# wangheda/youtube-8m

Hardware: AMD Instinct MI355X
Metric: training videos/sec (higher is better)
Workload: dtype f32; 1 GPU; BASELINE configs[3]: LstmModel (2 x BasicLSTMCell(1024), dynamic_rnn over F=300) on raw uint8 [B,300,1152] frames + MoeModel head (2 mixtures, V=4716), fp32 training step (fwd+bwd+clip+Adam); per_gpu_batch=128, global_batch=128, frames=300, parallelism=dp1, params=113902808

## Files before the change

### include/yt8m_hip.h

```cpp
#ifndef YT8M_HIP_H
#define YT8M_HIP_H
#include <stdint.h>

#ifdef __cplusplus
extern "C" {
#endif

typedef void* yt8m_stream_t;

enum yt8m_status { YT8M_OK = 0, YT8M_E_BADARG = -1, YT8M_E_SHAPE = -2, YT8M_E_HIP = -3, YT8M_E_RCCL = -4 };
enum yt8m_label_dtype { YT8M_LABEL_U8 = 0, YT8M_LABEL_F32 = 1 };

int yt8m_abi_version(void);
const char* yt8m_last_error(void);
const char* yt8m_built_arch(void);

int yt8m_prof_enable(int on);
int yt8m_prof_reset(void);
int yt8m_prof_get(int family, int64_t* launches, double* total_ms);
int yt8m_prof_get_flops(int family, double* flops);
int yt8m_prof_get_bytes(int family, double* bytes);

int yt8m_probe_mfma_f32(int iters, int blocks, float* sink, yt8m_stream_t stream);
int yt8m_probe_mfma_bf16(int iters, int blocks, int random_operands, float* sink, yt8m_stream_t stream);
int yt8m_probe_copy_f32(const float* src, float* dst, int64_t n, yt8m_stream_t stream);
int yt8m_probe_placement(int* out, int blocks, int spin_ticks, yt8m_stream_t stream);
int yt8m_stream_create_cu_mask(const uint32_t* mask, int words, yt8m_stream_t* stream);
int yt8m_stream_destroy(yt8m_stream_t stream);

int yt8m_gemm_f32(int transA, int transB, int64_t M, int64_t N, int64_t K,
                  const float* A, int64_t lda, const float* B, int64_t ldb,
                  float* C, int64_t ldc, const float* bias, float beta, yt8m_stream_t stream);

int yt8m_gemm_f32_batched(int transA, int transB, int64_t M, int64_t N, int64_t K,
                          const float* A, int64_t lda, int64_t strideA, const float* B, int64_t ldb, int64_t strideB,
                          float* C, int64_t ldc, int64_t strideC, float beta, int64_t batch, yt8m_stream_t stream);

typedef struct yt8m_gemm_problem {
  int64_t M, N, K;
  const void* A; int64_t lda;
  const void* B; int64_t ldb;
  float* C; int64_t ldc;
  const float* bias;
  float beta;
} yt8m_gemm_problem;
int64_t yt8m_gemm_workspace_bytes(void);
int yt8m_gemm_f32_grouped(int transA, int transB, int nprob, const yt8m_gemm_problem* probs, void* workspace,
                          int64_t workspace_bytes, yt8m_stream_t stream);
int yt8m_gemm_bf16_nt_grouped(int nprob, const yt8m_gemm_problem* probs, void* workspace, int64_t workspace_bytes,
                              yt8m_stream_t stream);
int64_t yt8m_x3_image_bytes(int64_t rows, int64_t K);
int yt8m_x3_split(const float* src, int64_t R, int64_t C, int64_t ld, float scale, void* plain, void* trans, yt8m_stream_t stream);
int yt8m_gemm_x3_nt_grouped(int nprob, const yt8m_gemm_problem* probs, void* workspace, int64_t workspace_bytes,
                            yt8m_stream_t stream);
int yt8m_h2_split(const float* src, int64_t R, int64_t C, int64_t ld, float scale, const float* dscale, void* plain, void* trans,
                  float* colpart, yt8m_stream_t stream);
int yt8m_h2_absmax(const float* src, int64_t R, int64_t C, int64_t ld, void* word, yt8m_stream_t stream);
int yt8m_h2_degraded(uint64_t* counts, int reset, yt8m_stream_t stream);
int yt8m_h2_split_dropout(const float* src, int64_t R, int64_t C, float scale, const float* dscale, void* plain, void* trans,
                          float keep_prob, uint64_t seed, int64_t offset, yt8m_stream_t stream);
int yt8m_h2_split_rowmax(const float* src, int64_t R, int64_t C, int64_t ld, const void* rowmax, float* inv, void* plain,
                         yt8m_stream_t stream);
int yt8m_h2_split_ex(const float* src, int64_t R, int64_t C, int64_t ld, float scale, const void* dscale, const float* rowscale, void* plain,
                     void* trans, void* trans_scaled, float* colpart, float* colpart_scaled, yt8m_stream_t stream);
int yt8m_gemm_h1x2_nt_ex(int64_t M, int64_t N, int64_t K, const void* A1, int64_t ska, const void* B2, int64_t skb, float* C, int64_t ldc,
                         const float* bias, float alpha, const void* dsb, const float* rowscale, const float* colsum, float colsum_scale,
                         float beta, void* workspace, int64_t workspace_bytes, yt8m_stream_t stream);
int yt8m_h2_rowscales(const float* src, int64_t R, int64_t C, int64_t ld, float* S, float* inv, yt8m_stream_t stream);
int yt8m_h2_split_rows(const float* src, int64_t R, int64_t C, int64_t ld, const float* S, void* plain, yt8m_stream_t stream);
int yt8m_gemm_h2_nt_ex(int64_t M, int64_t N, int64_t K, const void* A2, int64_t ska, const void* B2, int64_t skb, float* C, int64_t ldc,
                       const float* bias, float alpha, const void* dsa, const void* dsb, const float* rowscale, float beta, void* workspace,
                       int64_t workspace_bytes, yt8m_stream_t stream);
int yt8m_timepool_max_f32(const float* y, int64_t F, int64_t B, int64_t N, int64_t ldy, float* out, int32_t* idx, int64_t ldo,
                          yt8m_stream_t stream);
int yt8m_timepool_shiftmax_f32(const float* z, int64_t F, int64_t B, int64_t ldz, int nfilt, const int32_t* fs, const int32_t* ncol, float* out,
                               int32_t* idx, int64_t ldo, yt8m_stream_t stream);
int yt8m_u8_cnn_pool_dw(const uint8_t* q, const float* r_tm, const int32_t* idx, const float* g, int64_t ldg, int64_t B, int64_t F, int64_t D,
                        int64_t N, int64_t fs, float* dW, float beta, yt8m_stream_t stream);
int yt8m_f32_cnn_pool_dw(const float* x, int64_t ldx, const int32_t* idx, const float* g, int64_t ldg, int64_t B, int64_t F, int64_t D,
                         int64_t N, int64_t fs, float* dW, int64_t lddw, float beta, yt8m_stream_t stream);
int yt8m_f32_cnn_pool_dx(const int32_t* idx, const float* g, int64_t ldg, int64_t B, int64_t F, int64_t D, int nfilt, const float* const* wt,
                         const int32_t* fs, const int32_t* ncol, float* dx, int64_t lddx, yt8m_stream_t stream);
int yt8m_u8_frames_image_f16(const uint8_t* q, const int32_t* num_frames, int64_t B, int64_t F, int64_t D, float eps, void* image,
                             float* x_tm, float* r_out, yt8m_stream_t stream);
int yt8m_u8_frames_image_t_f16(const uint8_t* q, const int32_t* num_frames, int64_t B, int64_t F, int64_t D, void* image_t,
                               yt8m_stream_t stream);
int yt8m_gemm_h2_nt_grouped(int nprob, const yt8m_gemm_problem* probs, const float* alphas, const float* const* dsa,
                            const float* const* dsb, void* workspace, int64_t workspace_bytes, yt8m_stream_t stream);
int yt8m_x3_set_combine(int mode);
int yt8m_x3_set_schedule(int mode);
#define YT8M_GEMM_ROLE_DW 0x100
#define YT8M_GEMM_ROLE_H2 0x200
int yt8m_gemm_x3_pays(int64_t M, int64_t N, int64_t K);
int64_t yt8m_gemm_auto_scratch_bytes(int transA, int transB, int nprob, const yt8m_gemm_problem* probs);
int yt8m_gemm_auto_grouped(int transA, int transB, int nprob, const yt8m_gemm_problem* probs, void* workspace,
                           int64_t workspace_bytes, void* image_scratch, int64_t image_scratch_bytes, uint64_t* used_x3,
                           yt8m_stream_t stream);
int yt8m_gemm_auto_grouped_ex(int transA, int transB, int nprob, const yt8m_gemm_problem* probs, const float* const* absmaxA,
                              const float* const* absmaxB, void* workspace, int64_t workspace_bytes, void* image_scratch,
                              int64_t image_scratch_bytes, uint64_t* used_x3, yt8m_stream_t stream);
int yt8m_gemm_x1x3_nt(int64_t M, int64_t N, int64_t K, const void* A1, const void* B3, float* C, int64_t ldc, const float* bias,
                      const float* rowscale, const float* colsum, float colsum_scale, void* workspace, int64_t workspace_bytes,
                      yt8m_stream_t stream);
int yt8m_gemm_x1x3_nt_ex(int64_t M, int64_t N, int64_t K, const void* A1, int64_t ska, const void* B3, int64_t skb, float* C,
                         int64_t ldc, const float* bias, float alpha, const float* rowscale, const float* colsum,
                         float colsum_scale, float beta, void* workspace, int64_t workspace_bytes, yt8m_stream_t stream);
int yt8m_bf16_image(const float* src, int64_t R, int64_t C, int64_t ld, float scale, void* plain, void* trans, yt8m_stream_t stream);
int yt8m_gemm_b1_nt_grouped(int nprob, const yt8m_gemm_problem* probs, void* workspace, int64_t workspace_bytes, yt8m_stream_t stream);
int yt8m_gemm_b1_nt_grouped_bf16c(int nprob, const yt8m_gemm_problem* probs, unsigned c_bf16_mask, void* workspace, int64_t workspace_bytes,
                                  yt8m_stream_t stream);
int yt8m_moe_mix_fwd_bf16z(const void* Zg, const void* Ze, float* p, int64_t B, int64_t V, int M, yt8m_stream_t stream);
int yt8m_moe_mix_bwd_bf16_images_z16(const void* Zg, const void* Ze, const float* dp, const void* labels, int label_dtype, int64_t B,
                                     int64_t V, int M, float eps, float dscale, const float* upstream_dev, void* dZg_img, int64_t g_kb,
                                     void* dZg_t_img, int64_t gt_kb, void* dZe_img, int64_t e_kb, void* dZe_t_img, int64_t et_kb,
                                     float* be_part, yt8m_stream_t stream);
int yt8m_bf16_image_colsum(const float* src, int64_t R, int64_t C, int64_t ld, float scale, const float* rowscale, void* plain,
                           void* trans, void* trans_scaled, float* colpart, float* colpart_scaled, yt8m_stream_t stream);
int yt8m_gemm_b1_nt_ex(int64_t M, int64_t N, int64_t K, const void* A1, int64_t ska, const void* B1, int64_t skb, float* C, int64_t ldc,
                       const float* bias, float alpha, const float* rowscale, const float* colsum, float colsum_scale, float beta,
                       void* workspace, int64_t workspace_bytes, yt8m_stream_t stream);
int yt8m_x3_split_ex(const float* src, int64_t R, int64_t C, int64_t ld, float scale, const float* rowscale, void* plain,
                     void* trans, void* trans_scaled, yt8m_stream_t stream);
int yt8m_x3_split_colsum(const float* src, int64_t R, int64_t C, int64_t ld, float scale, const float* rowscale, void* plain,
                         void* trans, void* trans_scaled, float* colpart, float* colpart_scaled, yt8m_stream_t stream);
int yt8m_cast_f32_bf16(const float* src, int64_t rows, int64_t cols, int64_t ld, void* dst, int64_t dst_ld, int transpose,
                       yt8m_stream_t stream);
int yt8m_cast_f32_bf16_dual(const float* src, int64_t rows, int64_t cols, int64_t ld, void* dst_plain, int64_t plain_ld,
                            void* dst_trans, int64_t trans_ld, yt8m_stream_t stream);

int yt8m_l2norm_fwd_f32(const float* x, float* y, int64_t rows, int64_t cols, float eps, yt8m_stream_t stream);
int yt8m_l2norm_bwd_f32(const float* x, const float* dy, float* dx, int64_t rows, int64_t cols, float eps,
                        yt8m_stream_t stream);
int yt8m_dequant_l2norm_u8(const uint8_t* q, const int32_t* num_frames, float* x,
                           int64_t B, int64_t F, int64_t D, float eps, yt8m_stream_t stream);
int yt8m_dequant_mean_l2norm_u8(const uint8_t* q, const int32_t* num_frames, float* x,
                                int64_t B, int64_t F, int64_t D, float eps, yt8m_stream_t stream);
int yt8m_resolution_mean_u8(const uint8_t* q, const int32_t* num_frames, float* y, int32_t* num_frames_out, int64_t B, int64_t F,
                            int64_t D, int64_t resolution, int l2norm, float eps, yt8m_stream_t stream);
int yt8m_resolution_mean_f32(const float* x, const int32_t* num_frames, float* y, int32_t* num_frames_out, int64_t B, int64_t F,
                             int64_t D, int64_t resolution, int l2norm, float eps, yt8m_stream_t stream);
int yt8m_frame_pyramid_u8(const uint8_t* q, const int32_t* num_frames, int64_t B, int64_t F, int64_t D, int levels, int nseg,
                          const int64_t* widths, float* const* y, int32_t* const* num_frames_out, float eps, yt8m_stream_t stream);
int yt8m_frame_pyramid_supported(int64_t D, int nseg, const int64_t* widths, int levels);

int yt8m_moe_mix_fwd(const float* Zg, const float* Ze, float* p, int64_t B, int64_t V, int M,
                     yt8m_stream_t stream);
int yt8m_moe_mix_bwd(float* Zg, float* Ze, const float* dp, int64_t B, int64_t V, int M,
                     yt8m_stream_t stream);

int64_t yt8m_moe_mix_xent_workspace_bytes(int64_t B, int64_t V);
int yt8m_moe_mix_xent_fwd(const float* Zg, const float* Ze, const void* labels, int label_dtype, float* p,
                          float* loss_out, int64_t B, int64_t V, int M, float eps, void* workspace,
                          yt8m_stream_t stream);
int yt8m_moe_mix_xent_bwd(float* Zg, float* Ze, const void* labels, int label_dtype, const float* upstream_dev,
                          int64_t B, int64_t V, int M, float eps, float upstream, yt8m_stream_t stream);
int yt8m_moe_mix_xent_bwd_absmax(float* Zg, float* Ze, const void* labels, int label_dtype, const float* upstream_dev, int64_t B, int64_t V,
                                 int M, float eps, float upstream, void* absmax2, yt8m_stream_t stream);

int64_t yt8m_moe_workspace_bytes(int64_t B, int64_t V);
int64_t yt8m_moe_workspace_bytes_ex(int64_t B, int64_t D, int64_t V, int M);
int yt8m_moe_fwd(const float* x, const float* Wg, const float* We, const float* be, const void* labels, int label_dtype,
                 int64_t B, int64_t D, int64_t V, int M, float eps, float* Zg, float* Ze, float* p, float* loss_out,
                 void* workspace, int64_t workspace_bytes, yt8m_stream_t stream);
int yt8m_moe_bwd(const float* x, const float* Wg, const float* We, float* Zg, float* Ze, const void* labels, int label_dtype,
                 int64_t B, int64_t D, int64_t V, int M, float eps, float upstream, float* dWg, float* dWe, float* dbe,
                 float beta, float* dx, void* workspace, int64_t workspace_bytes, yt8m_stream_t stream);
int yt8m_logistic_fwd_bwd(const float* x, const float* W, const float* b, const void* labels, int label_dtype, int64_t B,
                          int64_t D, int64_t V, float eps, float* p, float* loss_out, float* Z, float* dW, float* db,
                          float beta, float* dx, void* workspace, int64_t workspace_bytes, yt8m_stream_t stream);

int yt8m_skinny_supported(int64_t M, int64_t K, int64_t N);
int64_t yt8m_skinny_workspace_bytes(int64_t M, int64_t K, int64_t N);
int yt8m_skinny_fwd_f32(const float* x, int64_t ldx, const float* W, int64_t ldw, const float* bias, float* y, int64_t ldy,
                        int64_t M, int64_t K, int64_t N, float beta, yt8m_stream_t stream);
int yt8m_skinny_dw_f32(const float* x, int64_t ldx, const float* dy, int64_t ldy, float* dW, int64_t lddw, int64_t M, int64_t K,
                       int64_t N, float beta, void* workspace, int64_t workspace_bytes, yt8m_stream_t stream);
int yt8m_skinny_dx_f32(const float* dy, int64_t ldy, const float* W, int64_t ldw, float* dx, int64_t lddx, int64_t M, int64_t K,
                       int64_t N, float beta, yt8m_stream_t stream);

int64_t yt8m_lstm_packed16_elems(int64_t B, int64_t H);
int yt8m_lstm_pack_bf16(const float* Wh, int64_t ldw, int64_t H, void* Wp16, void* Wq16, yt8m_stream_t stream);
int yt8m_lstm_steps_fwd_bf16(float* z, const void* Wp16, float* cs, float* hs, void* hs16, float* out, const int32_t* num_frames,
                             int64_t t0, int64_t T, int64_t B, int64_t H, float forget_bias, yt8m_stream_t stream);
// ... 409 lines not shown
```

### youtube-8m_amd/_lib.py

```python
import ctypes
import os

_HERE = os.path.dirname(os.path.abspath(__file__))
LIB_PATH = os.environ.get("YT8M_LIB", os.path.join(_HERE, "libyt8m_hip.so"))

c_void_p, c_int, c_int64, c_float, c_double = ctypes.c_void_p, ctypes.c_int, ctypes.c_int64, ctypes.c_float, ctypes.c_double
P = c_void_p

class GemmProblem(ctypes.Structure):
    _fields_ = [("M", c_int64), ("N", c_int64), ("K", c_int64), ("A", c_void_p), ("lda", c_int64), ("B", c_void_p),
                ("ldb", c_int64), ("C", c_void_p), ("ldc", c_int64), ("bias", c_void_p), ("beta", c_float)]


STREAM_HOOK = ctypes.CFUNCTYPE(None, ctypes.c_void_p, ctypes.c_void_p)


class PersistBwdImages(ctypes.Structure):
    _fields_ = [("plain", ctypes.c_void_p), ("trans", ctypes.c_void_p), ("trans_scaled", ctypes.c_void_p), ("rowscale", ctypes.c_void_p),
                ("colpart", ctypes.c_void_p), ("colpart_scaled", ctypes.c_void_p)]


class LstmStackDesc(ctypes.Structure):
    _fields_ = [("B", c_int64), ("F", c_int64), ("D", c_int64), ("H", c_int64), ("L", ctypes.c_int32), ("input_u8", ctypes.c_int32),
                ("forget_bias", c_float), ("fwd_chunks", ctypes.c_int32), ("bwd_chunks", ctypes.c_int32), ("need_dx", ctypes.c_int32),
                ("input_keep_prob", c_float), ("reserved0", ctypes.c_int32), ("dropout_seed", ctypes.c_uint64 * 8)]


class WimgDemand(ctypes.Structure):
    _fields_ = [("src", c_void_p), ("R", c_int64), ("C", c_int64), ("ld", c_int64), ("trans", ctypes.c_int32), ("planes", ctypes.c_int32),
                ("scale", c_float), ("pad", ctypes.c_int32)]


class WimgSpec(ctypes.Structure):
    _fields_ = [("plain", c_void_p), ("trans", c_void_p), ("row0", c_int64), ("rows", c_int64), ("scale", c_float),
                ("planes", ctypes.c_int32)]


class WimgJob(ctypes.Structure):
    _fields_ = [("offset", c_int64), ("R", c_int64), ("C", c_int64), ("tensor", ctypes.c_int32), ("nspec", ctypes.c_int32),
                ("tile_base", c_int64), ("spec", WimgSpec * 4)]


class OptRanges(ctypes.Structure):
    _fields_ = [("w", c_void_p), ("m", c_void_p), ("v", c_void_p), ("g", c_void_p), ("chunks", c_void_p), ("tensor_chunk_start", c_void_p),
                ("tensor_chunk_start_host", c_void_p), ("l2", c_void_p), ("partial", c_void_p), ("norms", c_void_p), ("skip_tensor", c_void_p),
                ("jobs", c_void_p), ("job_tensor_host", c_void_p), ("job_tile_base_host", c_void_p), ("njobs", ctypes.c_int32),
                ("nranges", ctypes.c_int32), ("range_lo", ctypes.c_int32 * 8), ("range_hi", ctypes.c_int32 * 8), ("gscale", c_float),
                ("clip", c_float), ("lr_t", c_float), ("beta1", c_float), ("beta2", c_float), ("eps", c_float), ("after_stream", c_void_p)]


DESC = ctypes.POINTER(LstmStackDesc)
PP = ctypes.POINTER(c_void_p)

SIGNATURES = {
    "yt8m_abi_version": (c_int, []),
    "yt8m_last_error": (ctypes.c_char_p, []),
    "yt8m_built_arch": (ctypes.c_char_p, []),
    "yt8m_prof_enable": (c_int, [c_int]),
    "yt8m_prof_reset": (c_int, []),
    "yt8m_prof_get": (c_int, [c_int, ctypes.POINTER(c_int64), ctypes.POINTER(c_double)]),
    "yt8m_prof_get_flops": (c_int, [c_int, ctypes.POINTER(c_double)]),
    "yt8m_prof_get_bytes": (c_int, [c_int, ctypes.POINTER(ctypes.c_double)]),
    "yt8m_probe_mfma_f32": (c_int, [c_int, c_int, P, P]),
    "yt8m_probe_mfma_bf16": (c_int, [c_int, c_int, c_int, P, P]),
    "yt8m_probe_copy_f32": (c_int, [P, P, c_int64, P]),
    "yt8m_probe_placement": (c_int, [P, c_int, c_int, P]),
    "yt8m_stream_create_cu_mask": (c_int, [P, c_int, ctypes.POINTER(P)]),
    "yt8m_stream_destroy": (c_int, [P]),
    "yt8m_gemm_f32": (c_int, [c_int, c_int, c_int64, c_int64, c_int64, P, c_int64, P, c_int64, P, c_int64, P, c_float, P]),
    "yt8m_gemm_workspace_bytes": (c_int64, []),
    "yt8m_gemm_f32_grouped": (c_int, [c_int, c_int, c_int, ctypes.POINTER(GemmProblem), P, c_int64, P]),
    "yt8m_gemm_bf16_nt_grouped": (c_int, [c_int, ctypes.POINTER(GemmProblem), P, c_int64, P]),
    "yt8m_gemm_x3_pays": (c_int, [c_int64, c_int64, c_int64]),
    "yt8m_gemm_auto_scratch_bytes": (c_int64, [c_int, c_int, c_int, ctypes.POINTER(GemmProblem)]),
    "yt8m_gemm_auto_grouped": (c_int, [c_int, c_int, c_int, ctypes.POINTER(GemmProblem), P, c_int64, P, c_int64, ctypes.POINTER(ctypes.c_uint64), P]),
    "yt8m_gemm_auto_grouped_ex": (c_int, [c_int, c_int, c_int, ctypes.POINTER(GemmProblem), ctypes.POINTER(ctypes.c_void_p), ctypes.POINTER(ctypes.c_void_p),
                                          P, c_int64, P, c_int64, ctypes.POINTER(ctypes.c_uint64), P]),
    "yt8m_x3_image_bytes": (c_int64, [c_int64, c_int64]),
    "yt8m_x3_split": (c_int, [P, c_int64, c_int64, c_int64, c_float, P, P, P]),
    "yt8m_gemm_x3_nt_grouped": (c_int, [c_int, ctypes.POINTER(GemmProblem), P, c_int64, P]),
    "yt8m_gemm_x1x3_nt": (c_int, [c_int64, c_int64, c_int64, P, P, P, c_int64, P, P, P, c_float, P, c_int64, P]),
    "yt8m_gemm_x1x3_nt_ex": (c_int, [c_int64, c_int64, c_int64, P, c_int64, P, c_int64, P, c_int64, P, c_float, P, P, c_float, c_float, P,
                                     c_int64, P]),
    "yt8m_bf16_image": (c_int, [P, c_int64, c_int64, c_int64, c_float, P, P, P]),
    "yt8m_gemm_b1_nt_grouped": (c_int, [c_int, ctypes.POINTER(GemmProblem), P, c_int64, P]),
    "yt8m_gemm_b1_nt_grouped_bf16c": (c_int, [c_int, ctypes.POINTER(GemmProblem), ctypes.c_uint, P, c_int64, P]),
    "yt8m_x3_split_ex": (c_int, [P, c_int64, c_int64, c_int64, c_float, P, P, P, P, P]),
    "yt8m_x3_split_colsum": (c_int, [P, c_int64, c_int64, c_int64, c_float, P, P, P, P, P, P, P]),
    "yt8m_x3_set_combine": (c_int, [c_int]),
    "yt8m_x3_set_schedule": (c_int, [c_int]),
    "yt8m_bf16_image_colsum": (c_int, [P, c_int64, c_int64, c_int64, c_float, P, P, P, P, P, P, P]),
    "yt8m_gemm_b1_nt_ex": (c_int, [c_int64, c_int64, c_int64, P, c_int64, P, c_int64, P, c_int64, P, c_float, P, P, c_float, c_float, P,
                                   c_int64, P]),
    "yt8m_u8_frames_image_t": (c_int, [P, P, c_int64, c_int64, c_int64, P, P]),
    "yt8m_lstm_stack_supported": (c_int, [DESC]),
    "yt8m_lstm_stack_tape_bytes": (c_int64, [DESC]),
    "yt8m_lstm_stack_scratch_bytes": (c_int64, [DESC]),
    "yt8m_lstm_stack_partition": (c_int, [DESC, ctypes.POINTER(c_int), ctypes.POINTER(c_int)]),
    "yt8m_lstm_stack_set_prep_hook": (c_int, [P, P]),
    "yt8m_lstm_stack_streams": (c_int, [c_int, PP, ctypes.POINTER(c_void_p)]),
    "yt8m_lstm_stack_fwd": (c_int, [DESC, P, P, PP, PP, P, c_int64, P, c_int64, P]),
    "yt8m_lstm_stack_view": (c_int, [DESC, P, c_int, c_int, ctypes.POINTER(c_void_p)]),
    "yt8m_lstm_stack_bwd": (c_int, [DESC, P, P, PP, P, c_int64, P, c_int64, P, PP, PP, PP, PP, ctypes.POINTER(c_float),
                                    ctypes.POINTER(c_float), P, P]),
    "yt8m_lstm_stack_status": (c_int, [DESC, P, P]),
    "yt8m_lstm_stack_layer_done_wait": (c_int, [c_int, P]),
    "yt8m_u8_frames_image": (c_int, [P, P, c_int64, c_int64, c_int64, c_float, P, P, P, P]),
    "yt8m_cast_f32_bf16": (c_int, [P, c_int64, c_int64, c_int64, P, c_int64, c_int, P]),
    "yt8m_cast_f32_bf16_dual": (c_int, [P, c_int64, c_int64, c_int64, P, c_int64, P, c_int64, P]),
    "yt8m_gemm_f32_batched": (c_int, [c_int, c_int, c_int64, c_int64, c_int64, P, c_int64, c_int64, P, c_int64, c_int64,
                                      P, c_int64, c_int64, c_float, c_int64, P]),
    "yt8m_l2norm_fwd_f32": (c_int, [P, P, c_int64, c_int64, c_float, P]),
    "yt8m_l2norm_bwd_f32": (c_int, [P, P, P, c_int64, c_int64, c_float, P]),
    "yt8m_dequant_l2norm_u8": (c_int, [P, P, P, c_int64, c_int64, c_int64, c_float, P]),
    "yt8m_dequant_mean_l2norm_u8": (c_int, [P, P, P, c_int64, c_int64, c_int64, c_float, P]),
    "yt8m_moe_workspace_bytes": (c_int64, [c_int64, c_int64]),
    "yt8m_moe_workspace_bytes_ex": (c_int64, [c_int64, c_int64, c_int64, c_int]),
    "yt8m_moe_fwd": (c_int, [P, P, P, P, P, c_int, c_int64, c_int64, c_int64, c_int, c_float, P, P, P, P, P, c_int64, P]),
    "yt8m_moe_bwd": (c_int, [P, P, P, P, P, P, c_int, c_int64, c_int64, c_int64, c_int, c_float, c_float, P, P, P, c_float, P, P,
                             c_int64, P]),
    "yt8m_logistic_fwd_bwd": (c_int, [P, P, P, P, c_int, c_int64, c_int64, c_int64, c_float, P, P, P, P, P, c_float, P, P,
                                      c_int64, P]),
    "yt8m_moe_mix_fwd": (c_int, [P, P, P, c_int64, c_int64, c_int, P]),
    "yt8m_moe_mix_bwd": (c_int, [P, P, P, c_int64, c_int64, c_int, P]),
    "yt8m_moe_mix_xent_workspace_bytes": (c_int64, [c_int64, c_int64]),
    "yt8m_moe_mix_xent_fwd": (c_int, [P, P, P, c_int, P, P, c_int64, c_int64, c_int, c_float, P, P]),
    "yt8m_moe_mix_xent_bwd": (c_int, [P, P, P, c_int, P, c_int64, c_int64, c_int, c_float, c_float, P]),
    "yt8m_moe_mix_xent_bwd_absmax": (c_int, [P, P, P, c_int, P, c_int64, c_int64, c_int, c_float, c_float, P, P]),
    "yt8m_skinny_supported": (c_int, [c_int64, c_int64, c_int64]),
    "yt8m_skinny_workspace_bytes": (c_int64, [c_int64, c_int64, c_int64]),
    "yt8m_skinny_fwd_f32": (c_int, [P, c_int64, P, c_int64, P, P, c_int64, c_int64, c_int64, c_int64, c_float, P]),
    "yt8m_skinny_dw_f32": (c_int, [P, c_int64, P, c_int64, P, c_int64, c_int64, c_int64, c_int64, c_float, P, c_int64, P]),
    "yt8m_skinny_dx_f32": (c_int, [P, c_int64, P, c_int64, P, c_int64, c_int64, c_int64, c_int64, c_float, P]),
    "yt8m_lstm_packed16_elems": (c_int64, [c_int64, c_int64]),
    "yt8m_lstm_pack_bf16": (c_int, [P, c_int64, c_int64, P, P, P]),
    "yt8m_lstm_steps_fwd_bf16": (c_int, [P, P, P, P, P, P, P, c_int64, c_int64, c_int64, c_int64, c_float, P]),
    "yt8m_lstm_steps_bwd_bf16": (c_int, [P, P, P, P, P, P, P, c_int, P, c_int64, c_int64, c_int64, c_int64, P]),
    "yt8m_u8_frame_scales": (c_int, [P, P, c_int64, c_int64, c_int64, c_float, P, P]),
    "yt8m_skinny_fwd_u8": (c_int, [P, c_int64, P, c_int64, P, P, P, P, c_int64, c_int64, c_int64, c_int64, c_float, P]),
    "yt8m_skinny_dw_u8": (c_int, [P, c_int64, P, c_int64, P, P, c_int64, c_int64, c_int64, c_int64, c_float, P, c_int64, P]),
    "yt8m_attn_pool_fwd_u8": (c_int, [P, P, P, P, c_int64, c_int64, c_int64, c_int64, P]),
    "yt8m_attn_pool_dw_u8": (c_int, [P, P, P, P, P, c_int64, c_int64, c_int64, c_int64, P]),
    "yt8m_attn_pool_supported": (c_int, [c_int64, c_int64, c_int64, c_int64]),
    "yt8m_attn_pool_fwd": (c_int, [P, P, P, c_int64, c_int64, c_int64, c_int64, P]),
    "yt8m_attn_pool_bwd": (c_int, [P, P, P, P, P, c_int64, c_int64, c_int64, c_int64, P]),
    "yt8m_gru_layer_fwd": (c_int, [P, P, P, c_int64, P, c_int64, P, P, P, P, c_int64, c_int64, c_int64, P, c_int64, P]),
    "yt8m_gru_layer_bwd": (c_int, [P, P, P, c_int64, P, c_int64, P, P, P, P, P, P, P, c_int64, c_int64, c_int64, P, c_int64, P]),
    "yt8m_lnlstm_layer_fwd": (c_int, [P, P, c_int64, P, P, P, P, P, P, P, c_int64, c_int64, c_int64, c_float, c_float,
                                      ctypes.c_uint64, P, c_int64, P]),
    "yt8m_lnlstm_layer_bwd": (c_int, [P, P, c_int64, P, P, P, P, P, P, P, P, P, P, P, P, c_int64, c_int64, c_int64, c_float,
                                      c_float, ctypes.c_uint64, P, c_int64, P]),
    "yt8m_dropout_f32": (c_int, [P, P, c_int64, c_float, ctypes.c_uint64, c_int64, P]),
    "yt8m_add_noise_f32": (c_int, [P, P, c_int64, c_float, ctypes.c_uint64, c_int64, P]),
    "yt8m_moe_mix_bwd_bf16_partial_rows": (c_int64, [c_int64]),
    "yt8m_moe_mix_bwd_bf16": (c_int, [P, P, P, P, c_int, c_int64, c_int64, c_int, c_float, c_float, P, P, c_int64, P, c_int64,
                                      P, c_int64, P, c_int64, P, P]),
    "yt8m_moe_mix_bwd_bf16_images": (c_int, [P, P, P, P, c_int, c_int64, c_int64, c_int, c_float, c_float, P, P, c_int64, P, c_int64,
                                      P, c_int64, P, c_int64, P, P]),
    "yt8m_moe_mix_bwd_bf16_images_z16": (c_int, [P, P, P, P, c_int, c_int64, c_int64, c_int, c_float, c_float, P, P, c_int64, P, c_int64,
                                      P, c_int64, P, c_int64, P, P]),
# ... 206 lines not shown
```

### youtube-8m_amd/csrc/gemm_auto.hip

```cpp
#include <stdlib.h>
#include <algorithm>
#include <vector>
#include "common.h"

using namespace yt8m;

namespace {

constexpr double X3_RATE = 195e12, F32_RATE = 110e12, SPLIT_RATE = 3.2e12;

bool image_form_pays(int64_t M, int64_t N, int64_t K, double rate_mul, double split_bytes) {
  if (M <= 0 || N <= 0 || K <= 0) return false;
  const double fl = 2.0 * (double)M * (double)N * (double)K;
  const int64_t tm = (M + 255) / 256, tn = (N + 255) / 256;
  const double eff = (double)M * (double)N / ((double)(tm * tn) * 65536.0);
  const double tiles = (double)(tm * tn);
  double occ = std::min(1.0, tiles * (double)std::max<int64_t>(1, std::min<int64_t>(8, K / 128)) / 256.0);
  if (occ < 1.0 && K >= 32768 && tiles >= 16.0) occ = std::max(occ, 0.7 * std::min(1.0, tiles * 16.0 / 256.0));
  const double tx3 = fl / (X3_RATE * rate_mul * eff * occ) + ((double)M * K + (double)N * K) * split_bytes / SPLIT_RATE + 2e-5;
  const double t32 = fl / (F32_RATE * std::min(1.0, (double)(((M + 127) / 128) * ((N + 127) / 128)) *
                                                        (double)std::max<int64_t>(1, std::min<int64_t>(8, K / 256)) / 768.0));
  return tx3 < 0.9 * t32;
}
bool x3_pays(int64_t M, int64_t N, int64_t K) { return image_form_pays(M, N, K, 1.0, 10.0); }

bool x3_allowed(const yt8m_gemm_problem& q, bool h2 = false) {
  static const bool off = getenv("YT8M_GEMM_X3") != nullptr && atoi(getenv("YT8M_GEMM_X3")) == 0;
  static const bool h2_price = !(getenv("YT8M_GEMM_H2_PRICE") != nullptr && atoi(getenv("YT8M_GEMM_H2_PRICE")) == 0);
  return !off && (q.beta == 0.f || q.beta == 1.f) && std::max(q.M, std::max(q.N, q.K)) < 64LL * 65535 &&
         ((h2 && h2_price) ? image_form_pays(q.M, q.N, q.K, 1.65, 8.0) : x3_pays(q.M, q.N, q.K));
}

int64_t up256(int64_t v) { return (v + 255) / 256 * 256; }

struct Img { const void* src; int64_t R, C, ld; bool trans; int64_t off; bool h2; const float* word; };

bool h2_role(int transA_flags, int transB, int64_t K) {
  static const bool off = getenv("YT8M_GEMM_H2") != nullptr && atoi(getenv("YT8M_GEMM_H2")) == 0;
  static const int64_t mink = getenv("YT8M_GEMM_H2_MINK") ? atoll(getenv("YT8M_GEMM_H2_MINK")) : 512;
  if (off || K < mink) return false;
  if ((transA_flags & YT8M_GEMM_ROLE_H2) != 0) return true;
  return (transA_flags & YT8M_GEMM_ROLE_DW) != 0 && (transA_flags & 1) != 0 && transB == 0;
}
constexpr int64_t H2_SCALE_BYTES = 256;

const void* resident(const void* src, int64_t R, int64_t C, int64_t ld, bool trans) {
  return yt8m_wimg_lookup(static_cast<const float*>(src), R, C, ld, trans ? 1 : 0, 3, 1.0f);
}

}

extern "C" int yt8m_gemm_x3_pays(int64_t M, int64_t N, int64_t K) { return x3_pays(M, N, K) ? 1 : 0; }

extern "C" int64_t yt8m_gemm_auto_scratch_bytes(int transA_flags, int transB, int nprob, const yt8m_gemm_problem* probs) {
  if (nprob < 1 || !probs) return 0;
  const int transA = transA_flags & 1;
  int64_t n = 0;
  for (int i = 0; i < nprob; ++i) {
    const yt8m_gemm_problem& q = probs[i];
    const bool h2q = h2_role(transA_flags, transB, q.K) && (q.N % 4) == 0;
    if (!x3_allowed(q, h2q)) continue;
    if (h2q) {
      if (!yt8m_wimg_lookup(static_cast<const float*>(q.A), transA ? q.K : q.M, transA ? q.M : q.K, q.lda, transA ? 1 : 0, 2, 0.0f))
        n += H2_SCALE_BYTES + up256(yt8m_x3_image_bytes(q.M, q.K));
      if (!yt8m_wimg_lookup(static_cast<const float*>(q.B), transB ? q.N : q.K, transB ? q.K : q.N, q.ldb, transB == 0 ? 1 : 0, 2, 0.0f))
        n += H2_SCALE_BYTES + up256(yt8m_x3_image_bytes(q.N, q.K));
      continue;
    }
    if (!resident(q.A, transA ? q.K : q.M, transA ? q.M : q.K, q.lda, transA != 0)) n += up256(yt8m_x3_image_bytes(q.M, q.K));
    if (!resident(q.B, transB ? q.N : q.K, transB ? q.K : q.N, q.ldb, transB == 0)) n += up256(yt8m_x3_image_bytes(q.N, q.K));
  }
  return n;
}

extern "C" int yt8m_gemm_auto_grouped(int transA_flags, int transB, int nprob, const yt8m_gemm_problem* probs, void* workspace,
                                      int64_t workspace_bytes, void* image_scratch, int64_t image_scratch_bytes, uint64_t* used_x3,
                                      yt8m_stream_t stream) {
  return yt8m_gemm_auto_grouped_ex(transA_flags, transB, nprob, probs, nullptr, nullptr, workspace, workspace_bytes, image_scratch,
                                   image_scratch_bytes, used_x3, stream);
}

extern "C" int yt8m_gemm_auto_grouped_ex(int transA_flags, int transB, int nprob, const yt8m_gemm_problem* probs, const float* const* absmaxA,
                                         const float* const* absmaxB, void* workspace, int64_t workspace_bytes, void* image_scratch,
                                         int64_t image_scratch_bytes, uint64_t* used_x3, yt8m_stream_t stream) {
  YT8M_REQUIRE(nprob >= 1 && nprob <= 64 && probs, YT8M_E_BADARG, "1..64 problems per call");
  YT8M_REQUIRE((transA_flags & ~(1 | YT8M_GEMM_ROLE_DW | YT8M_GEMM_ROLE_H2)) == 0 && (transB & ~1) == 0, YT8M_E_BADARG,
               "transA: 0 / 1 (| YT8M_GEMM_ROLE_DW | YT8M_GEMM_ROLE_H2), transB: 0 / 1");
  const int transA = transA_flags & 1;
  YT8M_REQUIRE((reinterpret_cast<uintptr_t>(image_scratch) & 255) == 0, YT8M_E_BADARG, "image scratch must be 256-byte aligned");
  std::vector<Img> imgs;
  std::vector<yt8m_gemm_problem> px, p32, ph;
  std::vector<const float*> hda, hdb;
  uint64_t mask = 0;
  int64_t off = 0;
  char* const base = static_cast<char*>(image_scratch);
  auto image_of = [&](const void* src, int64_t R, int64_t C, int64_t ld, bool trans, bool h2, const float* ext, const void** at,
                      const float** word) -> bool {
    if (!h2)
      if (const void* r = resident(src, R, C, ld, trans)) { *at = r; return true; }
    if (h2 && !ext)
      if (const void* r = yt8m_wimg_lookup(static_cast<const float*>(src), R, C, ld, trans ? 1 : 0, 2, 0.0f)) {
        *at = r;
        *word = reinterpret_cast<const float*>(static_cast<const char*>(r) - H2_SCALE_BYTES);
        return true;
      }
    for (const Img& m : imgs)
      if (m.src == src && m.R == R && m.C == C && m.ld == ld && m.trans == trans && m.h2 == h2) {
        *at = base + m.off;
        *word = m.word ? m.word : reinterpret_cast<const float*>(base + m.off - H2_SCALE_BYTES);
        return true;
      }
    const int64_t bytes = up256(trans ? yt8m_x3_image_bytes(C, R) : yt8m_x3_image_bytes(R, C)) + (h2 ? H2_SCALE_BYTES : 0);
    if (!image_scratch || off + bytes > image_scratch_bytes) return false;
    imgs.push_back({src, R, C, ld, trans, off + (h2 ? H2_SCALE_BYTES : 0), h2, h2 ? ext : nullptr});
    *at = base + off + (h2 ? H2_SCALE_BYTES : 0);
    *word = (h2 && ext) ? ext : reinterpret_cast<const float*>(base + off);
    off += bytes;
    return true;
  };
  for (int i = 0; i < nprob; ++i) {
    const yt8m_gemm_problem& q = probs[i];
    const bool h2 = h2_role(transA_flags, transB, q.K) && (q.N % 4) == 0;
    bool x3 = q.M > 0 && q.N > 0 && x3_allowed(q, h2) && q.A && q.B;
    const void* ia = nullptr;
    const void* ib = nullptr;
    const float* wa = nullptr;
    const float* wb = nullptr;
    if (x3) {
      const int64_t mark = off;
      const size_t nimg = imgs.size();
      x3 = image_of(q.A, transA ? q.K : q.M, transA ? q.M : q.K, q.lda, transA != 0, h2, absmaxA ? absmaxA[i] : nullptr, &ia, &wa) &&
           image_of(q.B, transB ? q.N : q.K, transB ? q.K : q.N, q.ldb, transB == 0, h2, absmaxB ? absmaxB[i] : nullptr, &ib, &wb);
      if (!x3) { imgs.resize(nimg); off = mark; }
    }
    if (x3) {
      yt8m_gemm_problem t = q;
      t.A = ia; t.lda = 0;
      t.B = ib; t.ldb = 0;
      if (h2) {
        ph.push_back(t);
        hda.push_back(wa);
        hdb.push_back(wb);
      } else {
        px.push_back(t);
      }
      mask |= 1ULL << i;
    } else {
      p32.push_back(q);
    }
  }
  for (const Img& m : imgs) {
    void* dst = static_cast<char*>(image_scratch) + m.off;
    int rc;
    if (m.h2) {
      const float* word = m.word;
      if (!word) {
        yt8m_wimg_note_demand(static_cast<const float*>(m.src), m.R, m.C, m.ld, m.trans ? 1 : 0, 2, 0.0f);
        float* w = reinterpret_cast<float*>(static_cast<char*>(dst) - H2_SCALE_BYTES);
        YT8M_HIP_CHECK(hipMemsetAsync(w, 0, 4, as_stream(stream)));
        rc = yt8m_h2_absmax(static_cast<const float*>(m.src), m.R, m.C, m.ld, w, stream);
        if (rc != YT8M_OK) return rc;
        word = w;
      }
      rc = yt8m_h2_split(static_cast<const float*>(m.src), m.R, m.C, m.ld, 1.0f, word, m.trans ? nullptr : dst, m.trans ? dst : nullptr, nullptr, stream);
    } else {
      rc = yt8m_x3_split(static_cast<const float*>(m.src), m.R, m.C, m.ld, 1.0f, m.trans ? nullptr : dst, m.trans ? dst : nullptr, stream);
    }
    if (rc != YT8M_OK) return rc;
  }
  for (size_t lo = 0; lo < ph.size(); lo += 4) {
    const int n = (int)std::min<size_t>(4, ph.size() - lo);
    int rc = yt8m_gemm_h2_nt_grouped(n, &ph[lo], nullptr, &hda[lo], &hdb[lo], workspace, workspace_bytes, stream);
    if (rc != YT8M_OK) return rc;
  }
  for (size_t lo = 0; lo < px.size(); lo += 4) {
    int rc = yt8m_gemm_x3_nt_grouped((int)std::min<size_t>(4, px.size() - lo), &px[lo], workspace, workspace_bytes, stream);
    if (rc != YT8M_OK) return rc;
  }
  for (size_t lo = 0; lo < p32.size(); lo += 4) {
    int rc = yt8m_gemm_f32_grouped(transA, transB, (int)std::min<size_t>(4, p32.size() - lo), &p32[lo], workspace, workspace_bytes, stream);
    if (rc != YT8M_OK) return rc;
  }
  if (used_x3) *used_x3 = mask;
  return YT8M_OK;
}
```

Baseline: 7971 videos/s.

## Add fused split-bf16x3 weight-gradient GEMM kernel for small-K accumulate problems

Adds a new grouped kernel for transposed-A weight-gradient GEMMs with K up to 128 (batch-row reductions) that reads fp32 operands directly, splits them into three bf16 planes in LDS on the fly, runs 32x32x16 bf16 MFMAs over six cross products, and accumulates into C. The auto-GEMM dispatcher routes qualifying DW problems (by default those with beta==1) to this path. This skips the separate x3/h2 image-split passes, their scratch traffic and the extra launches for these gradients. The trade-off is a persistent grid capped at 2x the CU count and a fixed 128x256 tile, which may underfill or load-balance worse than the existing path on some shapes.

Result: no change. 8020 videos/s, median of 6 (+0.6%).

```diff
diff --git a/include/yt8m_hip.h b/include/yt8m_hip.h
--- a/include/yt8m_hip.h
+++ b/include/yt8m_hip.h
@@ -99,6 +99,9 @@
 int yt8m_gemm_auto_grouped_ex(int transA, int transB, int nprob, const yt8m_gemm_problem* probs, const float* const* absmaxA,
                               const float* const* absmaxB, void* workspace, int64_t workspace_bytes, void* image_scratch,
                               int64_t image_scratch_bytes, uint64_t* used_x3, yt8m_stream_t stream);
+int yt8m_gemm_rows128_set(int mode);
+int yt8m_gemm_rows128_dw_takes(int transA, int transB, const yt8m_gemm_problem* prob);
+int yt8m_gemm_rows128_dw_grouped(int nprob, const yt8m_gemm_problem* probs, yt8m_stream_t stream);
 int yt8m_gemm_x1x3_nt(int64_t M, int64_t N, int64_t K, const void* A1, const void* B3, float* C, int64_t ldc, const float* bias,
                       const float* rowscale, const float* colsum, float colsum_scale, void* workspace, int64_t workspace_bytes,
                       yt8m_stream_t stream);
diff --git a/youtube-8m_amd/_lib.py b/youtube-8m_amd/_lib.py
--- a/youtube-8m_amd/_lib.py
+++ b/youtube-8m_amd/_lib.py
@@ -76,6 +76,9 @@
     "yt8m_gemm_auto_grouped": (c_int, [c_int, c_int, c_int, ctypes.POINTER(GemmProblem), P, c_int64, P, c_int64, ctypes.POINTER(ctypes.c_uint64), P]),
     "yt8m_gemm_auto_grouped_ex": (c_int, [c_int, c_int, c_int, ctypes.POINTER(GemmProblem), ctypes.POINTER(ctypes.c_void_p), ctypes.POINTER(ctypes.c_void_p),
                                           P, c_int64, P, c_int64, ctypes.POINTER(ctypes.c_uint64), P]),
+    "yt8m_gemm_rows128_set": (c_int, [c_int]),
+    "yt8m_gemm_rows128_dw_takes": (c_int, [c_int, c_int, ctypes.POINTER(GemmProblem)]),
+    "yt8m_gemm_rows128_dw_grouped": (c_int, [c_int, ctypes.POINTER(GemmProblem), P]),
     "yt8m_x3_image_bytes": (c_int64, [c_int64, c_int64]),
     "yt8m_x3_split": (c_int, [P, c_int64, c_int64, c_int64, c_float, P, P, P]),
     "yt8m_gemm_x3_nt_grouped": (c_int, [c_int, ctypes.POINTER(GemmProblem), P, c_int64, P]),
diff --git a/youtube-8m_amd/csrc/gemm_auto.hip b/youtube-8m_amd/csrc/gemm_auto.hip
--- a/youtube-8m_amd/csrc/gemm_auto.hip
+++ b/youtube-8m_amd/csrc/gemm_auto.hip
@@ -58,6 +58,7 @@
   int64_t n = 0;
   for (int i = 0; i < nprob; ++i) {
     const yt8m_gemm_problem& q = probs[i];
+    if (yt8m_gemm_rows128_dw_takes(transA_flags, transB, &q)) continue;
     const bool h2q = h2_role(transA_flags, transB, q.K) && (q.N % 4) == 0;
     if (!x3_allowed(q, h2q)) continue;
     if (h2q) {
@@ -89,7 +90,7 @@
   const int transA = transA_flags & 1;
   YT8M_REQUIRE((reinterpret_cast<uintptr_t>(image_scratch) & 255) == 0, YT8M_E_BADARG, "image scratch must be 256-byte aligned");
   std::vector<Img> imgs;
-  std::vector<yt8m_gemm_problem> px, p32, ph;
+  std::vector<yt8m_gemm_problem> px, p32, ph, pr;
   std::vector<const float*> hda, hdb;
   uint64_t mask = 0;
   int64_t off = 0;
@@ -120,6 +121,11 @@
   };
   for (int i = 0; i < nprob; ++i) {
     const yt8m_gemm_problem& q = probs[i];
+    if (yt8m_gemm_rows128_dw_takes(transA_flags, transB, &q)) {
+      pr.push_back(q);
+      mask |= 1ULL << i;
+      continue;
+    }
     const bool h2 = h2_role(transA_flags, transB, q.K) && (q.N % 4) == 0;
     bool x3 = q.M > 0 && q.N > 0 && x3_allowed(q, h2) && q.A && q.B;
     const void* ia = nullptr;
@@ -168,6 +174,10 @@
     }
     if (rc != YT8M_OK) return rc;
   }
+  for (size_t lo = 0; lo < pr.size(); lo += 4) {
+    int rc = yt8m_gemm_rows128_dw_grouped((int)std::min<size_t>(4, pr.size() - lo), &pr[lo], stream);
+    if (rc != YT8M_OK) return rc;
+  }
   for (size_t lo = 0; lo < ph.size(); lo += 4) {
     const int n = (int)std::min<size_t>(4, ph.size() - lo);
     int rc = yt8m_gemm_h2_nt_grouped(n, &ph[lo], nullptr, &hda[lo], &hdb[lo], workspace, workspace_bytes, stream);
diff --git a/youtube-8m_amd/csrc/gemm_rows128.hip b/youtube-8m_amd/csrc/gemm_rows128.hip
--- /dev/null
+++ b/youtube-8m_amd/csrc/gemm_rows128.hip
@@ -0,0 +1,258 @@
+#include <stdlib.h>
+#include <algorithm>
+#include <atomic>
+#include "common.h"
+
+using namespace yt8m;
+
+namespace {
+
+constexpr int TM = 128, TN = 256;
+constexpr int GA = TM / 4 + 4, GB = TN / 4 + 4;
+constexpr int PLANE_A = 4 * GA * 8, PLANE_B = 4 * GB * 8;
+constexpr int OFF_B = 3 * PLANE_A;
+constexpr int STAGE_F = 3 * (PLANE_A + PLANE_B);
+constexpr int LDS_BYTES = 2 * STAGE_F * 4;
+constexpr int P = 68;
+
+typedef float f32x16 __attribute__((ext_vector_type(16)));
+typedef float f32x2 __attribute__((ext_vector_type(2)));
+typedef __bf16 bf16x8 __attribute__((ext_vector_type(8)));
+typedef __bf16 bf16x2 __attribute__((ext_vector_type(2)));
+
+struct DwArgs {
+  const float* A;
+  const float* B;
+  float* C;
+  int64_t lda, ldb, ldc;
+  int M, N, K;
+  int tiles_m;
+  int tile_base;
+  int accumulate;
+};
+struct DwGroup {
+  DwArgs p[4];
+  int nprob;
+  int tiles;
+};
+
+__device__ __forceinline__ unsigned pk_bf16(float a, float b) {
+  const f32x2 v = {a, b};
+  return __builtin_bit_cast(unsigned, __builtin_convertvector(v, bf16x2));
+}
+__device__ __forceinline__ bool finite_bits(float x) { return (__float_as_uint(x) & 0x7F800000u) != 0x7F800000u; }
+__device__ __forceinline__ void split8(const float (&x)[8], uint4& p0, uint4& p1, uint4& p2) {
+  unsigned w[3][4];
+#pragma unroll
+  for (int t = 0; t < 4; ++t) {
+    const float a = x[2 * t], b = x[2 * t + 1];
+    const unsigned h1 = pk_bf16(a, b);
+    float ra = finite_bits(a) ? a - __uint_as_float(h1 << 16) : 0.f;
+    float rb = finite_bits(b) ? b - __uint_as_float(h1 & 0xFFFF0000u) : 0.f;
+    const unsigned h2 = pk_bf16(ra, rb);
+    ra -= __uint_as_float(h2 << 16);
+    rb -= __uint_as_float(h2 & 0xFFFF0000u);
+    w[0][t] = h1;
+    w[1][t] = h2;
+    w[2][t] = pk_bf16(ra, rb);
+  }
+  p0 = make_uint4(w[0][0], w[0][1], w[0][2], w[0][3]);
+  p1 = make_uint4(w[1][0], w[1][1], w[1][2], w[1][3]);
+  p2 = make_uint4(w[2][0], w[2][1], w[2][2], w[2][3]);
+}
+
+__global__ __launch_bounds__(256) __attribute__((amdgpu_waves_per_eu(2, 2))) void rows128_dw_kernel(const DwGroup G) {
+  extern __shared__ __attribute__((aligned(16))) float smem[];
+  for (int bid = (int)blockIdx.x; bid < G.tiles; bid += (int)gridDim.x) {
+  int q = 0;
+  for (int i = 1; i < G.nprob; ++i)
+    if (bid >= G.p[i].tile_base) q = i;
+  const DwArgs& g = G.p[q];
+  const int lt = bid - g.tile_base;
+  const int m0 = (lt % g.tiles_m) * TM, n0 = (lt / g.tiles_m) * TN;
+  const int tid = threadIdx.x, lane = tid & 63, wave = tid >> 6;
+  const int li = lane & 31, lk = lane >> 5;
+  const int wn = wave * 64;
+  const int nk = (g.K + 15) >> 4;
+
+  const bool isA = tid < 64;
+  const int u = isA ? tid : tid - 64;
+  const int cq = u >> 1, kh = u & 1;
+  const int col = (isA ? m0 : n0) + 4 * cq;
+  const bool live = tid < 192 && col < (isA ? g.M : g.N);
+  const int64_t ld = isA ? g.lda : g.ldb;
+  const float* src = (isA ? g.A : g.B) + (live ? col : 0);
+  const int plane = isA ? PLANE_A : PLANE_B;
+  const int grp = isA ? GA * 8 : GB * 8;
+  const int soff = (isA ? 0 : OFF_B) + cq * 8;
+
+  float4 v[8];
+  auto fetch = [&](int kt) __attribute__((always_inline)) {
+#pragma unroll
+    for (int j = 0; j < 8; ++j) {
+      const int k = kt * 16 + kh * 8 + j;
+      v[j] = *reinterpret_cast<const float4*>(src + (int64_t)min(k, g.K - 1) * ld);
+    }
+  };
+  auto stash = [&](int kt, float* S) __attribute__((always_inline)) {
+    if (tid >= 192) return;
+#pragma unroll
+    for (int c = 0; c < 4; ++c) {
+      float x[8];
+#pragma unroll
+      for (int j = 0; j < 8; ++j) {
+        const float e = c == 0 ? v[j].x : (c == 1 ? v[j].y : (c == 2 ? v[j].z : v[j].w));
+        x[j] = (live && kt * 16 + kh * 8 + j < g.K) ? e : 0.f;
+      }
+      uint4 p0, p1, p2;
+      split8(x, p0, p1, p2);
+      float* d = S + soff + c * grp + 4 * (kh ^ (c >> 1));
+      *reinterpret_cast<uint4*>(d) = p0;
+      *reinterpret_cast<uint4*>(d + plane) = p1;
+      *reinterpret_cast<uint4*>(d + 2 * plane) = p2;
+    }
+  };
+
+  f32x16 acc[2][4];
+#pragma unroll
+  for (int j = 0; j < 2; ++j)
+#pragma unroll
+    for (int i = 0; i < 4; ++i)
+#pragma unroll
+      for (int r = 0; r < 16; ++r) acc[j][i][r] = 0.f;
+
+  const int fsw = 4 * (lk ^ ((li >> 1) & 1));
+  const int fa = (li & 3) * (GA * 8) + (li >> 2) * 8 + fsw;
+  const int fb = OFF_B + (li & 3) * (GB * 8) + ((wn >> 2) + (li >> 2)) * 8 + fsw;
+
+  fetch(0);
+  stash(0, smem);
+  __syncthreads();
+  for (int kt = 0; kt < nk; ++kt) {
+    const float* S = smem + (kt & 1) * STAGE_F;
+    const bool more = kt + 1 < nk;
+    bf16x8 xb[3][2];
+#pragma unroll
+    for (int p = 0; p < 3; ++p)
+#pragma unroll
+      for (int j = 0; j < 2; ++j) xb[p][j] = __builtin_bit_cast(bf16x8, *reinterpret_cast<const float4*>(&S[fb + p * PLANE_B + j * 64]));
+#pragma unroll
+    for (int pa = 2; pa >= 0; --pa) {
+      bf16x8 ya[4];
+#pragma unroll
+      for (int i = 0; i < 4; ++i) ya[i] = __builtin_bit_cast(bf16x8, *reinterpret_cast<const float4*>(&S[fa + pa * PLANE_A + i * 64]));
+#pragma unroll
+      for (int pb = 2 - pa; pb >= 0; --pb)
+#pragma unroll
+        for (int i = 0; i < 4; ++i)
+#pragma unroll
+          for (int j = 0; j < 2; ++j) acc[j][i] = __builtin_amdgcn_mfma_f32_32x32x16_bf16(xb[pb][j], ya[i], acc[j][i], 0, 0, 0);
+      if (pa == 2) {
+        __builtin_amdgcn_sched_barrier(0);
+        fetch(kt + 1);
+        __builtin_amdgcn_sched_barrier(0);
+      }
+    }
+    __builtin_amdgcn_sched_barrier(0);
+    if (more) stash(kt + 1, smem + ((kt + 1) & 1) * STAGE_F);
+    __syncthreads();
+  }
+
+  float* st = smem + wave * (32 * P);
+#pragma unroll
+  for (int i = 0; i < 4; ++i) {
+#pragma unroll
+    for (int j = 0; j < 2; ++j)
+#pragma unroll
+      for (int c = 0; c < 4; ++c)
+        *reinterpret_cast<float4*>(&st[li * P + 32 * j + 8 * c + 4 * lk]) =
+            make_float4(acc[j][i][4 * c], acc[j][i][4 * c + 1], acc[j][i][4 * c + 2], acc[j][i][4 * c + 3]);
+    __syncthreads();
+    float4 t[8];
+#pragma unroll
+    for (int rr = 0; rr < 8; ++rr) t[rr] = *reinterpret_cast<const float4*>(&st[(rr * 4 + (lane >> 4)) * P + (lane & 15) * 4]);
+    if (g.accumulate) {
+      float4 old[8];
+#pragma unroll
+      for (int rr = 0; rr < 8; ++rr) {
+        const int gm = min(m0 + 32 * i + rr * 4 + (lane >> 4), g.M - 1), gn = min(n0 + wn + (lane & 15) * 4, g.N - 4);
+        old[rr] = *reinterpret_cast<const float4*>(g.C + (int64_t)gm * g.ldc + gn);
+      }
+#pragma unroll
+      for (int rr = 0; rr < 8; ++rr) { t[rr].x += old[rr].x; t[rr].y += old[rr].y; t[rr].z += old[rr].z; t[rr].w += old[rr].w; }
+    }
+#pragma unroll
+    for (int rr = 0; rr < 8; ++rr) {
+      const int gm = m0 + 32 * i + rr * 4 + (lane >> 4), gn = n0 + wn + (lane & 15) * 4;
+      if (gm < g.M && gn < g.N) *reinterpret_cast<float4*>(g.C + (int64_t)gm * g.ldc + gn) = t[rr];
+    }
+    __syncthreads();
+  }
+  }
+}
+
+std::atomic<int> g_mode{0};
+
+bool enabled(float beta) {
+  static const int env = getenv("YT8M_GEMM_ROWS128") ? atoi(getenv("YT8M_GEMM_ROWS128")) : -1;
+  const int m = g_mode.load(std::memory_order_relaxed);
+  if (m != 0) return m == 1;
+  return env < 0 ? beta == 1.f : env != 0;
+}
+
+bool aligned16(const void* p) { return (reinterpret_cast<uintptr_t>(p) & 15) == 0; }
+
+bool dw_shape_ok(const yt8m_gemm_problem& q) {
+  return q.M > 0 && q.N > 0 && q.K >= 16 && q.K <= 128 && (q.M % 4) == 0 && (q.N % 4) == 0 && q.M < (1LL << 30) && q.N < (1LL << 30) &&
+         q.A && q.B && q.C && !q.bias && (q.beta == 0.f || q.beta == 1.f) && (q.lda % 4) == 0 && (q.ldb % 4) == 0 && (q.ldc % 4) == 0 &&
+         q.lda >= q.M && q.ldb >= q.N && q.ldc >= q.N && aligned16(q.A) && aligned16(q.B) && aligned16(q.C) &&
+         ((q.M + TM - 1) / TM) * ((q.N + TN - 1) / TN) < (1LL << 28);
+}
+
+}
+
+extern "C" int yt8m_gemm_rows128_set(int mode) {
+  YT8M_REQUIRE(mode >= 0 && mode <= 2, YT8M_E_BADARG, "mode: 0 (process default), 1 (on), 2 (off)");
+  g_mode.store(mode, std::memory_order_relaxed);
+  return YT8M_OK;
+}
+
+extern "C" int yt8m_gemm_rows128_dw_takes(int transA_flags, int transB, const yt8m_gemm_problem* q) {
+  return (q && enabled(q->beta) && (transA_flags & 1) != 0 && (transA_flags & YT8M_GEMM_ROLE_DW) != 0 && transB == 0 && dw_shape_ok(*q)) ? 1 : 0;
+}
+
+extern "C" int yt8m_gemm_rows128_dw_grouped(int nprob, const yt8m_gemm_problem* probs, yt8m_stream_t stream) {
+  YT8M_REQUIRE(nprob >= 1 && nprob <= 4 && probs, YT8M_E_BADARG, "1..4 problems per call");
+  DwGroup G;
+  memset(&G, 0, sizeof(G));
+  int64_t tiles = 0;
+  double fl = 0.0;
+  for (int i = 0; i < nprob; ++i) {
+    const yt8m_gemm_problem& q = probs[i];
+    YT8M_REQUIRE(dw_shape_ok(q), YT8M_E_BADARG,
+                 "16 <= K <= 128, M % 4 == 0, N % 4 == 0, 16-byte aligned operands and pitches, no bias, beta 0 or 1");
+    DwArgs& a = G.p[i];
+    a.A = static_cast<const float*>(q.A);
+    a.B = static_cast<const float*>(q.B);
+    a.C = q.C;
+    a.lda = q.lda; a.ldb = q.ldb; a.ldc = q.ldc;
+    a.M = (int)q.M; a.N = (int)q.N; a.K = (int)q.K;
+    a.tiles_m = (int)((q.M + TM - 1) / TM);
+    a.tile_base = (int)tiles;
+    a.accumulate = q.beta != 0.f;
+    tiles += (int64_t)a.tiles_m * ((q.N + TN - 1) / TN);
+    fl += 2.0 * (double)q.M * (double)q.N * (double)q.K;
+  }
+  YT8M_REQUIRE(tiles < (1LL << 30), YT8M_E_SHAPE, "too many tiles");
+  G.nprob = nprob;
+  G.tiles = (int)tiles;
+  int dev = 0, cus = 0;
+  YT8M_HIP_CHECK(hipGetDevice(&dev));
+  YT8M_HIP_CHECK(hipDeviceGetAttribute(&cus, hipDeviceAttributeMultiprocessorCount, dev));
+  const unsigned grid = (unsigned)std::min<int64_t>(tiles, 2 * (int64_t)std::max(cus, 1));
+  static DeviceOnce once;
+  YT8M_HIP_CHECK(once.lds(reinterpret_cast<const void*>(&rows128_dw_kernel), LDS_BYTES));
+  ProfScope prof(F_GEMM_X3, as_stream(stream), fl);
+  hipLaunchKernelGGL(rows128_dw_kernel, dim3(grid), dim3(256), LDS_BYTES, as_stream(stream), G);
+  return launch_status("rows128_dw_kernel");
+}
```
